# psklavos1/adaptive-city-nerf

Measured on AMD Instinct MI355X. Metric: ray-samples/sec + PSNR, 4096 rays×256 samples, 1/2/4/8 MI355X, higher is better.
Workload: dtype f32; 1 GPU; c2; samples_per_ray=256, parallelism=ray-sharded x1

## Files before the change

### adaptive_city_nerf_amd/csrc/render.hip

```cpp
#include "acn_device.h"
#include "acn_internal.h"

using namespace acn;

#ifndef ACN_MLP_F16X3
#define ACN_MLP_F16X3 1
#endif

#ifndef ACN_SLOTS
#define ACN_SLOTS 1
#endif

#ifndef ACN_XPAIR
#define ACN_XPAIR 2
#endif
#ifndef ACN_LEVEL_PARITY
#define ACN_LEVEL_PARITY 0
#endif
#ifndef ACN_FINE_POL
#define ACN_FINE_POL 0
#endif
#ifndef ACN_FINE_FROM
#define ACN_FINE_FROM 8
#endif
// ... 978 lines not shown
                   [&](int, float px, float py, float pz, const float (&shv)[8], uint32_t& folded, float& yr, float& yg,
                       float& yb, float& ys) {
                       container_tile<INTERP, ROUTE, FOLD>(cfg, W, px, py, pz, shv, cb, &folded, lane, yr, yg, yb, ys);
                   });
    }
}

#ifndef ACN_RENDER_WS
#define ACN_RENDER_WS 1
#endif
constexpr int kWsMaxS = 256;
#ifndef ACN_WS_CHECK
#define ACN_WS_CHECK 0
#endif
#ifndef ACN_WS_PREFOLD
#define ACN_WS_PREFOLD 1
#endif
#ifndef ACN_WS_DTILE
#define ACN_WS_DTILE (ACN_WS_CHECK ? 0 : 8)
#endif

__device__ __forceinline__ void composite_ray_lds(const RenderParams& p, const BgArgs& bg, int64_t ray,
                                                  const f32x4* __restrict__ ys, int lane, float step) {
    const int j = lane & 31, h = lane >> 5;
    const int S = p.S;
    const float* rq = p.rays + ray * 8;
    const float dx = rq[3], dy = rq[4], dz = rq[5];
    const float near = rq[6], far = rq[7];
    const float* jit = p.jitter ? p.jitter + ray * S : nullptr;
    RayAcc acc{1.0, 0.0f, 0.0f, 0.0f, 0.0f, 0.0f};
    for (int s0 = 0; s0 < S; s0 += 32) {
        const int s = s0 + j;
        const bool valid = s < S;
        const int sc = valid ? s : S - 1;
        float t, dist;
        if (!jit) {
            const int i0 = sc < S - 1 ? sc : S - 2;
            const float ta = tlin_sel(near, far, i0, S, step), tb = tlin_sel(near, far, i0 + 1, S, step);
            t = sc < S - 1 ? ta : tb;
            dist = tb - ta;
        } else {
            t = tval(near, far, sc, S, jit);
            const float tn = (sc < S - 1) ? tval(near, far, sc + 1, S, jit) : t;
            const float tp = (sc == S - 1 && S > 1) ? tval(near, far, sc - 1, S, jit) : t;
            dist = (sc < S - 1) ? (tn - t) : (t - tp);
        }
        const f32x4 y = ys[sc];
        const float cr = clamp_nan(y[0], 0.0f, 1.0f);
        const float cg = clamp_nan(y[1], 0.0f, 1.0f);
        const float cbl = clamp_nan(y[2], 0.0f, 1.0f);
        float sig = clamp_min_nan(y[3], 0.0f);
        if (p.sigma_scale != 1.0f) sig = sig * p.sigma_scale;
        float wv;
        composite_tile(acc, valid, cr, cg, cbl, sig, t, dist, j, &wv);
        if (p.weights && valid && h == 0) p.weights[ray * S + s] = wv;
    }
    float bgc[3];
    background(bg, dx, dy, dz, lane, bgc);
    float r, g, b, dd, a;
    finish_ray(acc, r, g, b, dd, a);
    if (lane == 0) {
        if (bg.mode != ACN_BG_NONE) {
            const float om = 1.0f - a;
            r = r + om * bgc[0];
            g = g + om * bgc[1];
            b = b + om * bgc[2];
        }
        p.rgb[ray * 3 + 0] = r;
        p.rgb[ray * 3 + 1] = g;
        p.rgb[ray * 3 + 2] = b;
        p.depth[ray] = dd;
        p.acc[ray] = a;
    }
}

template <int INTERP>
__global__ void __launch_bounds__(1024, 4) render_ws_kernel(FieldCfg cfg, BgArgs bg, RenderParams p) {
    constexpr bool FOLD = ACN_SHFOLD != 0;
    __shared__ __attribute__((aligned(16))) float smem[PK_FLOATS];
    __shared__ __attribute__((aligned(16))) float cbuf[FOLD ? 16 * 64 : 4];
    __shared__ __attribute__((aligned(16))) f32x4 ybuf[16 * kWsMaxS];
    __shared__ int qhead;
    __shared__ int done[16];
    stage_weights<1>(smem, p.packed);
    const float* W = smem;
    const int wave = __builtin_amdgcn_readfirstlane(threadIdx.x >> 6);
    float* cb = FOLD ? cbuf + wave * 64 : nullptr;
    const int S = p.S;
    const int T = (S + 31) >> 5;
    const float step = 1.0f / (float)(S - 1);
    int64_t base, hi, stride;
    if ((gridDim.x & 7) == 0) {
        const int64_t chunk = (p.N + 7) >> 3;
        const int64_t lo = min(p.N, (int64_t)(blockIdx.x & 7) * chunk);
        hi = min(p.N, lo + chunk);
        base = lo + (int64_t)(blockIdx.x >> 3) * 16;
        stride = (int64_t)(gridDim.x >> 3) * 16;
    } else {
        hi = p.N;
        base = (int64_t)blockIdx.x * 16;
        stride = (int64_t)gridDim.x * 16;
    }
    for (; base < hi; base += stride) {
        const int tid = opaque_v((int)threadIdx.x);
        const int lane = tid & 63, j = lane & 31, h = lane >> 5;
        const float kz = __int_as_float(opaque_s(0));
        const int nr = (int)min((int64_t)16, hi - base);
        if (tid == 0) qhead = 0;
        if (tid < 16) done[tid] = 0;
        constexpr bool PRE = FOLD && ACN_WS_PREFOLD;
        if (PRE && wave < nr) {
            const int64_t r0 = p.order ? (int64_t)__builtin_amdgcn_readfirstlane(p.order[base + wave]) : base + wave;
            const float* rp = p.rays + r0 * 8;
            float sh[16], sv[8];
            dir_sh(rp[3], rp[4], rp[5], sh, kz);
            sh_rows_for_half(sh, h, sv);
            fold_sh_bias(W, sv, lane, cbuf + wave * 64);
        }
        __syncthreads();
#if ACN_WS_DTILE
        static_assert(!ACN_WS_DTILE || (FOLD && ACN_WS_PREFOLD && !ACN_WS_CHECK), "depth tiles read the pre-folded bias");
        static_assert(16 % (ACN_WS_DTILE > 0 ? ACN_WS_DTILE : 1) == 0, "ACN_WS_DTILE: rays per tile divide 16");
        {
            constexpr int R = ACN_WS_DTILE, D = 32 / R, NG = 16 / R;
            const int ND = (S + D - 1) / D;
            const float shz[8] = {0.0f, 0.0f, 0.0f, 0.0f, 0.0f, 0.0f, 0.0f, 0.0f};
            int gcur = -1;
            int slot = 0;
            float ox = 0.0f, oy = 0.0f, oz = 0.0f, dx = 0.0f, dy = 0.0f, dz = 0.0f, near = 0.0f, far = 0.0f;
            const float* jit = nullptr;
            for (;;) {
                int item = 0;
                if (lane == 0) item = __hip_atomic_fetch_add(&qhead, 1, __ATOMIC_RELAXED, __HIP_MEMORY_SCOPE_WORKGROUP);
                item = __builtin_amdgcn_readlane(item, 0);
                if (item >= NG * ND) break;
                const int g = NG == 1 ? 0 : item % NG, q = NG == 1 ? item : item / NG;
                if (g != gcur) {
                    slot = g * R + (j % R);
                    const int ls = slot < nr ? slot : nr - 1;
                    const int64_t ray = p.order ? (int64_t)p.order[base + ls] : base + ls;
                    const float* rp = p.rays + ray * 8;
                    ox = rp[0], oy = rp[1], oz = rp[2], dx = rp[3], dy = rp[4], dz = rp[5];
                    near = rp[6], far = rp[7];
                    jit = p.jitter ? p.jitter + ray * S : nullptr;
                    gcur = g;
                }
                const int s = q * D + j / R;
                const int sc = s < S ? s : S - 1;
                float t;
                if (!jit) {
                    const int i0 = sc < S - 1 ? sc : S - 2;
                    const float ta = tlin_sel(near, far, i0, S, step), tb = tlin_sel(near, far, i0 + 1, S, step);
                    t = sc < S - 1 ? ta : tb;
                } else {
                    t = tval(near, far, sc, S, jit);
                }
                const float px = ox + dx * t, py = oy + dy * t, pz = oz + dz * t;
                uint32_t fl = 1u;
                float yr, yg, yb, ys;
                container_tile<INTERP, 0, FOLD>(cfg, W, px, py, pz, shz, cbuf + slot * 64, &fl, lane, yr, yg, yb, ys);
                if (h == 0 && s < S && slot < nr) {
                    f32x4 v;
                    v[0] = yr, v[1] = yg, v[2] = yb, v[3] = ys;
                    ybuf[slot * kWsMaxS + s] = v;
                }
            }
            __syncthreads();
            if (wave < nr) {
                const int64_t ray_w = p.order ? (int64_t)__builtin_amdgcn_readfirstlane(p.order[base + wave]) : base + wave;
                composite_ray_lds(p, bg, ray_w, ybuf + wave * kWsMaxS, lane, step);
            }
            __syncthreads();
            continue;
        }
#endif
        int64_t cur = -1;
        uint32_t folded = 0u;
        float shv[8] = {0.0f, 0.0f, 0.0f, 0.0f, 0.0f, 0.0f, 0.0f, 0.0f};
        float ox = 0.0f, oy = 0.0f, oz = 0.0f, dx = 0.0f, dy = 0.0f, dz = 0.0f, near = 0.0f, far = 0.0f;
        const float* jit = nullptr;
        for (;;) {
            int item = 0;
            if (lane == 0) item = __hip_atomic_fetch_add(&qhead, 1, __ATOMIC_RELAXED, __HIP_MEMORY_SCOPE_WORKGROUP);
            item = __builtin_amdgcn_readlane(item, 0);
            if (item >= nr * T) break;
            const int tile = item / nr, slot = item - tile * nr;
            const int64_t ray = p.order ? (int64_t)__builtin_amdgcn_readfirstlane(p.order[base + slot]) : base + slot;
            if (ray != cur) {
                const float* rp = p.rays + ray * 8;
                ox = rp[0], oy = rp[1], oz = rp[2], dx = rp[3], dy = rp[4], dz = rp[5];
                near = rp[6], far = rp[7];
                jit = p.jitter ? p.jitter + ray * S : nullptr;
                if (!PRE || ACN_WS_CHECK) {
                    float sh[16];
                    dir_sh(dx, dy, dz, sh, kz);
                    sh_rows_for_half(sh, h, shv);
                    if (!PRE) folded = 0u;
                }
                cur = ray;
            }
            if (PRE) {
                cb = cbuf + slot * 64;
                folded = 1u;
            }
            const int s = tile * 32 + j;
            const int sc = s < S ? s : S - 1;
            float t;
            if (!jit) {
                const int i0 = sc < S - 1 ? sc : S - 2;
                const float ta = tlin_sel(near, far, i0, S, step), tb = tlin_sel(near, far, i0 + 1, S, step);
                t = sc < S - 1 ? ta : tb;
            } else {
                t = tval(near, far, sc, S, jit);
            }
            const float px = ox + dx * t, py = oy + dy * t, pz = oz + dz * t;
            float yr, yg, yb, ys;
            container_tile<INTERP, 0, FOLD>(cfg, W, px, py, pz, shv, cb, &folded, lane, yr, yg, yb, ys);
#if ACN_WS_CHECK
            {
                float cr, cg, cbb, cs;
                field_tile<INTERP, false, true>(W, cfg.ex[0], cfg.log2T, px, py, pz, shv, nullptr, lane, cr, cg, cbb, cs);
                cs = trunc_exp(cs);
                if (__float_as_uint(cr) != __float_as_uint(yr) || __float_as_uint(cg) != __float_as_uint(yg) ||
                    __float_as_uint(cbb) != __float_as_uint(yb) || __float_as_uint(cs) != __float_as_uint(ys))
                    yr = __int_as_float(0x7fc00000);
            }
#endif
            if (h == 0 && s < S) {
                f32x4 v;
                v[0] = yr, v[1] = yg, v[2] = yb, v[3] = ys;
                ybuf[slot * kWsMaxS + s] = v;
            }
            int old = 0;
            if (lane == 0) old = __hip_atomic_fetch_add(&done[slot], 1, __ATOMIC_ACQ_REL, __HIP_MEMORY_SCOPE_WORKGROUP);
            old = __builtin_amdgcn_readlane(old, 0);
            if (old != T - 1) continue;
            composite_ray_lds(p, bg, ray, ybuf + slot * kWsMaxS, lane, step);
        }
        __syncthreads();
    }
}

#ifndef ACN_SLOTS_SINGLE
#define ACN_SLOTS_SINGLE 1
#endif
constexpr uint32_t kSingleRay = 1u << 31;
__device__ __forceinline__ void soft_route_bits(const FieldCfg& cfg, float px, float py, float pz, uint32_t& m,
                                                bool& exact) {
    float mins = INFINITY;
    for (int k = 0; k < cfg.K; ++k) mins = fminf(mins, route_dist2(cfg, k, px, py, pz));
    float mind = sqrtf(mins);
    mind = mind < 1e-6f ? 1e-6f : mind;
    const float thr = cfg.bm * mind, thr2 = route_thr2(thr);
// ... 973 lines not shown
    Keval = active_module >= 0 ? 1 : K;
    ACN_REQUIRE(workspace && workspace_bytes >= (size_t)Keval * PK_BYTES, "workspace too small: need %zu bytes",
                (size_t)Keval * PK_BYTES);
    ACN_REQUIRE(((uintptr_t)workspace & 15) == 0, "workspace must be 16-byte aligned");
    interp = experts[k0].interp;
    const int log2T = experts[k0].log2T;
    PackArgs pa{};
    for (int i = 0; i < Keval; ++i) {
        const acn_expert& e = experts[k0 + i];
        int st = check_expert(e, k0 + i);
        if (st) return st;
        if (e.interp != interp || e.log2T != log2T)
            return acn_set_error(ACN_ERR_UNSUPPORTED, "experts must share interpolation and log2_hashmap_size");
        ExpertMeta& m = cfg.ex[i];
        m.table = e.table;
        for (int a = 0; a < 3; ++a) {
            m.amin[a] = e.aabb_min[a];
            m.ext[a] = e.aabb_extent[a];
            m.rext[a] = 1.0f / e.aabb_extent[a];
        }
        for (int l = 0; l < 16; ++l) m.res[l] = e.res[l];
        pa.e[i] = PackSrc{e.sig_w0, e.sig_b0, e.sig_w1, e.sig_b1, e.sigh_w, e.sigh_b, e.geo_w, e.geo_b,
                          e.col_w0, e.col_b0, e.col_w1, e.col_b1, e.col_w2, e.col_b2};
    }
    cfg.K = Keval;
    cfg.log2T = log2T;
    cfg.cluster_2d = routing->cluster_2d;
    cfg.bm = routing->boundary_margin;
    if (active_module >= 0 || K == 1) cfg.routing = 0;
    else cfg.routing = routing->boundary_margin > 1.0f ? 1 : 2;
    for (int k = 0; k < K && active_module < 0; ++k)
        for (int a = 0; a < 3; ++a) cfg.cent[k][a] = routing->centroids[k][a];
    if (do_pack) {
        hipLaunchKernelGGL(pack_kernel, dim3((PK_FLOATS + 255) / 256, Keval), dim3(256), 0, s, pa, Keval,
                           (float*)workspace);
        return acn_check_launch("acn_pack_experts");
    }
    return ACN_OK;
}

}

#define ACN_DISPATCH_I(L, I)                                           \
    do {                                                               \
        if (cfg.routing == 0) L(I, 1, 0);                              \
        else if (cfg.routing == 1) { if (K == 2) L(I, 2, 1); else L(I, 0, 1); } \
        else { if (K == 2) L(I, 2, 2); else L(I, 0, 2); }              \
    } while (0)
#define ACN_DISPATCH(L)                                                \
    do {                                                               \
        if (interp == 1) ACN_DISPATCH_I(L, 1);                         \
        else if (interp == 0) ACN_DISPATCH_I(L, 0);                    \
        else ACN_DISPATCH_I(L, 2);                                     \
    } while (0)

__global__ void __launch_bounds__(256) sample_train_kernel(const float* __restrict__ rays, int64_t N, int S,
                                                           const float* __restrict__ jit, float3 amin, float3 ext,
                                                           float lo, float hi, float* __restrict__ t_out,
                                                           float* __restrict__ x01, float* __restrict__ sh_out) {
    const int64_t m = (int64_t)blockIdx.x * 256 + threadIdx.x;
    if (m >= N * (int64_t)S) return;
    const int64_t ray = m / S;
    const int s = (int)(m - ray * S);
    const float* rp = rays + ray * 8;
    const float ox = rp[0], oy = rp[1], oz = rp[2], dx = rp[3], dy = rp[4], dz = rp[5];
    const float t = tval(rp[6], rp[7], s, S, jit ? jit + ray * S : nullptr);
    t_out[m] = t;
    const float px = ox + dx * t, py = oy + dy * t, pz = oz + dz * t;
    x01[m * 3 + 0] = clamp_nan((px - amin.x) / ext.x, lo, hi);
    x01[m * 3 + 1] = clamp_nan((py - amin.y) / ext.y, lo, hi);
    x01[m * 3 + 2] = clamp_nan((pz - amin.z) / ext.z, lo, hi);
    float sh[16];
    dir_sh(dx, dy, dz, sh);
    float4* o4 = reinterpret_cast<float4*>(sh_out + m * 16);
#pragma unroll
    for (int q = 0; q < 4; ++q) o4[q] = make_float4(sh[4 * q], sh[4 * q + 1], sh[4 * q + 2], sh[4 * q + 3]);
}

#define ACN_ORDER_MAX 8192
#define ACN_ORDER_BINS 4096
#ifndef ACN_ORDER_COUNTING
#define ACN_ORDER_COUNTING 1
#endif
__device__ __forceinline__ uint32_t spread6(uint32_t v) {
    v &= 63u;
    v = (v | (v << 4)) & 0x30Fu;
    v = (v | (v << 2)) & 0x333u;
    v = (v | (v << 1)) & 0x555u;
    return v;
}
template <int OP>
__device__ __forceinline__ float wave_reduce(float v) {
    auto op = [](float a, float b) { return OP == 0 ? a + b : fmaxf(a, b); };
    v = op(v, __int_as_float(__builtin_amdgcn_update_dpp(0, __float_as_int(v), 0xB1, 0xF, 0xF, false)));
    v = op(v, __int_as_float(__builtin_amdgcn_update_dpp(0, __float_as_int(v), 0x4E, 0xF, 0xF, false)));
    v = op(v, __int_as_float(__builtin_amdgcn_update_dpp(0, __float_as_int(v), 0x141, 0xF, 0xF, false)));
    v = op(v, __int_as_float(__builtin_amdgcn_update_dpp(0, __float_as_int(v), 0x140, 0xF, 0xF, false)));
    const float r0 = __int_as_float(__builtin_amdgcn_readlane(__float_as_int(v), 0));
    const float r1 = __int_as_float(__builtin_amdgcn_readlane(__float_as_int(v), 16));
    const float r2 = __int_as_float(__builtin_amdgcn_readlane(__float_as_int(v), 32));
    const float r3 = __int_as_float(__builtin_amdgcn_readlane(__float_as_int(v), 48));
    return op(op(r0, r1), op(r2, r3));
}
template <int OP>
__device__ __forceinline__ void block_reduce3(float& a, float& b, float& c, float* red) {
    a = wave_reduce<OP>(a), b = wave_reduce<OP>(b), c = wave_reduce<OP>(c);
    const int w = threadIdx.x >> 6;
    if ((threadIdx.x & 63) == 0) red[w] = a, red[16 + w] = b, red[32 + w] = c;
    __syncthreads();
    a = red[0], b = red[16], c = red[32];
    for (int k = 1; k < 16; ++k) a += red[k], b += red[16 + k], c += red[32 + k];
    __syncthreads();
}
__device__ __forceinline__ void block_reduce4max(float& a, float& b, float& c, float& d, float* red) {
    a = wave_reduce<1>(a), b = wave_reduce<1>(b), c = wave_reduce<1>(c), d = wave_reduce<1>(d);
    const int w = threadIdx.x >> 6;
    if ((threadIdx.x & 63) == 0) red[w] = a, red[16 + w] = b, red[32 + w] = c, red[48 + w] = d;
    __syncthreads();
    for (int k = 0; k < 16; ++k)
        a = fmaxf(a, red[k]), b = fmaxf(b, red[16 + k]), c = fmaxf(c, red[32 + k]), d = fmaxf(d, red[48 + k]);
    __syncthreads();
}
__device__ __forceinline__ bool dir_ok(float x, float y, float z) {
    const float n2 = x * x + y * y + z * z;
    return n2 > 0.0f && n2 < 3.0e38f;
}
template <bool FINAL>
__device__ __forceinline__ void radix_pass6(const uint16_t* kin, const uint16_t* iin, int shift, int N, int* cnt,
                                            int* wsum, uint16_t* kout, uint16_t* iout, int32_t* __restrict__ order) {
    const int tid = threadIdx.x, w = tid >> 6, lane = tid & 63;
    const int B = (((N + 15) >> 4) + 63) & ~63;
    const int lo = w * B, hi = min(N, lo + B);
    cnt[tid] = 0;
    __syncthreads();
    for (int p0 = lo; p0 < hi; p0 += 64) {
        const int pos = p0 + lane;
        const bool v = pos < hi;
        const int dig = v ? (kin[pos] >> shift) & 63 : 0;
        const uint64_t m = same_digit_lanes(v, dig);
        if (v && lanes_below(m) == 0) cnt[dig * 16 + w] += __popcll(m);
    }
    __syncthreads();
    const int val = cnt[tid];
    const int incl = wave_incl_scan(val);
    if (lane == 63) wsum[w] = incl;
    __syncthreads();
    int base = incl - val;
    for (int k = 0; k < w; ++k) base += wsum[k];
    cnt[tid] = base;
    __syncthreads();
    for (int p0 = lo; p0 < hi; p0 += 64) {
        const int pos = p0 + lane;
        const bool v = pos < hi;
        const uint16_t key = v ? kin[pos] : (uint16_t)0;
        const int dig = (key >> shift) & 63;
        const uint64_t m = same_digit_lanes(v, dig);
        const int below = lanes_below(m);
        const int run = v ? cnt[dig * 16 + w] : 0;
        if (v) {
            const int dst = run + below;
            const int idx = iin ? (int)iin[pos] : pos;
            if (FINAL) {
                order[dst] = idx;
            } else {
                kout[dst] = key;
                iout[dst] = (uint16_t)idx;
            }
        }
        if (v && below == 0) cnt[dig * 16 + w] = run + __popcll(m);
    }
    __syncthreads();
}
__global__ void __launch_bounds__(1024) ray_order_kernel(const float* __restrict__ rays, int N,
                                                         int32_t* __restrict__ order) {
    constexpr int PER = ACN_ORDER_MAX / 1024;
    __shared__ int cnt[1024];
    __shared__ __attribute__((aligned(16))) float dir[3][ACN_ORDER_MAX];
    __shared__ uint16_t cell_of[ACN_ORDER_MAX];
    __shared__ int wsum[16];
    __shared__ float red[16 * 4];
    const int tid = threadIdx.x;
    float sx = 0.0f, sy = 0.0f, sz = 0.0f;
#pragma unroll
    for (int q = 0; q < PER; ++q) {
        const int i = tid + q * 1024;
        if (i < N) {
            const float* rp = rays + (int64_t)i * 8;
            const float x = rp[3], y = rp[4], z = rp[5];
            dir[0][i] = x, dir[1][i] = y, dir[2][i] = z;
            if (dir_ok(x, y, z)) {
                const float r = rsqrtf(x * x + y * y + z * z);
                sx += x * r, sy += y * r, sz += z * r;
            }
        }
    }
#if ACN_ORDER_DIAG == 3
    for (int i = tid; i < N; i += 1024) order[i] = i + (int)(sx * 0.0f);
    return;
#endif
    block_reduce3<0>(sx, sy, sz, red);
    const float mn = sqrtf(sx * sx + sy * sy + sz * sz);
    float mx = 0.0f, my = 0.0f, mz = 1.0f;
    if (mn > 0.0f && mn < 3.0e38f) mx = sx / mn, my = sy / mn, mz = sz / mn;
    float ax = 0.0f, ay = 0.0f, az = 0.0f;
    if (fabsf(mx) <= fabsf(my) && fabsf(mx) <= fabsf(mz)) ax = 1.0f;
    else if (fabsf(my) <= fabsf(mz)) ay = 1.0f;
    else az = 1.0f;
    float e1x = my * az - mz * ay, e1y = mz * ax - mx * az, e1z = mx * ay - my * ax;
    const float e1n = rsqrtf(e1x * e1x + e1y * e1y + e1z * e1z);
    e1x *= e1n, e1y *= e1n, e1z *= e1n;
    const float e2x = my * e1z - mz * e1y, e2y = mz * e1x - mx * e1z, e2z = mx * e1y - my * e1x;
    auto coords = [&](int i, float& u, float& v) -> bool {
        const float x = dir[0][i], y = dir[1][i], z = dir[2][i];
        if (!dir_ok(x, y, z)) return false;
        const float dm = x * mx + y * my + z * mz;
        if (!(dm > 0.0f)) return false;
        u = (x * e1x + y * e1y + z * e1z) / dm;
        v = (x * e2x + y * e2y + z * e2z) / dm;
        return fabsf(u) < 1.0e30f && fabsf(v) < 1.0e30f;
    };
    float umin = 3.0e38f, vmin = 3.0e38f, umax = -3.0e38f, vmax = -3.0e38f;
    float cu[PER], cv[PER];
    bool cok[PER];
#pragma unroll
    for (int q = 0; q < PER; ++q) {
        const int i = tid + q * 1024;
        cok[q] = i < N && coords(i, cu[q], cv[q]);
        if (cok[q]) umin = fminf(umin, cu[q]), umax = fmaxf(umax, cu[q]), vmin = fminf(vmin, cv[q]), vmax = fmaxf(vmax, cv[q]);
    }
#if ACN_ORDER_DIAG == 2
    for (int i = tid; i < N; i += 1024) order[i] = i + (int)(umin * 0.0f + umax * 0.0f);
    return;
#endif
#if ACN_ORDER_DIAG == 1
    umin = -2.0f, vmin = -2.0f, umax = 2.0f, vmax = 2.0f;
#else
    umin = -umin, vmin = -vmin;
    block_reduce4max(umin, vmin, umax, vmax, red);
    umin = -umin, vmin = -vmin;
#endif
    const float su = umax > umin ? 63.999f / (umax - umin) : 0.0f;
    const float sv = vmax > vmin ? 63.999f / (vmax - vmin) : 0.0f;
#pragma unroll
    for (int q = 0; q < PER; ++q) {
        const int i = tid + q * 1024;
        if (i >= N) break;
        int c = ACN_ORDER_BINS - 1;
        if (cok[q]) {
            const uint32_t qu = (uint32_t)fminf(fmaxf((cu[q] - umin) * su, 0.0f), 63.0f);
            const uint32_t qv = (uint32_t)fminf(fmaxf((cv[q] - vmin) * sv, 0.0f), 63.0f);
            c = (int)(spread6(qu) | (spread6(qv) << 1));
        }
        cell_of[i] = (uint16_t)c;
    }
    __syncthreads();
#if ACN_ORDER_COUNTING
    {
        constexpr int kOrderSlice = 64;
        int* bins = reinterpret_cast<int*>(&dir[2][0]);
        int* start = reinterpret_cast<int*>(&dir[1][0]);
        uint16_t* lst = reinterpret_cast<uint16_t*>(&dir[0][0]);
        __shared__ int maxc;
        if (tid == 0) maxc = 0;
        for (int b = tid; b < ACN_ORDER_BINS; b += 1024) bins[b] = 0;
        __syncthreads();
        int mloc = 0;
        for (int i = tid; i < N; i += 1024) {
            const int c = atomicAdd(&bins[cell_of[i]], 1) + 1;
            mloc = c > mloc ? c : mloc;
        }
        if (mloc > kOrderSlice) atomicMax(&maxc, mloc);
        __syncthreads();
        if (maxc == 0) {
            constexpr int BPT = ACN_ORDER_BINS / 1024;
            int c[BPT], tot = 0;
#pragma unroll
            for (int q = 0; q < BPT; ++q) tot += (c[q] = bins[tid * BPT + q]);
            const int lane = tid & 63, w = tid >> 6;
            const int incl = wave_incl_scan(tot);
            if (lane == 63) wsum[w] = incl;
            __syncthreads();
            int base = incl - tot;
            for (int k = 0; k < w; ++k) base += wsum[k];
#pragma unroll
            for (int q = 0; q < BPT; ++q) {
                start[tid * BPT + q] = base;
                bins[tid * BPT + q] = base;
                base += c[q];
            }
            __syncthreads();
            for (int i = tid; i < N; i += 1024) lst[atomicAdd(&bins[cell_of[i]], 1)] = (uint16_t)i;
            __syncthreads();
            for (int i = tid; i < N; i += 1024) {
                const int cl = cell_of[i], s0 = start[cl], s1 = bins[cl];
                int r = 0;
                for (int j = s0; j < s1; ++j) r += (int)lst[j] < i ? 1 : 0;
                order[s0 + r] = i;
            }
            return;
        }
        __syncthreads();
    }
#endif
    uint16_t* key1 = reinterpret_cast<uint16_t*>(&dir[0][0]);
    uint16_t* idx1 = reinterpret_cast<uint16_t*>(&dir[1][0]);
    radix_pass6<false>(cell_of, nullptr, 0, N, cnt, wsum, key1, idx1, nullptr);
    radix_pass6<true>(key1, idx1, 6, N, cnt, wsum, nullptr, nullptr, order);
}

extern "C" size_t acn_workspace_bytes(int K) { return (size_t)(K < 1 ? 1 : K) * PK_BYTES; }

extern "C" size_t acn_render_order_bytes(int64_t N) {
    if (N < 1) return 0;
    return N <= ACN_ORDER_MAX ? (size_t)N * sizeof(int32_t) : 0;
}

extern "C" int acn_ray_order(const float* rays, int64_t N, int32_t* order, void* stream) {
    ACN_REQUIRE(N >= 1 && N <= ACN_ORDER_MAX, "acn_ray_order: N must be in [1, %d], got %lld", ACN_ORDER_MAX,
                (long long)N);
    ACN_REQUIRE(rays && order, "acn_ray_order: NULL pointer");
    hipLaunchKernelGGL(ray_order_kernel, dim3(1), dim3(1024), 0, (hipStream_t)stream, rays, (int)N, order);
    return acn_check_launch("acn_ray_order");
}

extern "C" int acn_pack_experts(const acn_expert* experts, const acn_routing* routing, int active_module,
                                void* workspace, size_t workspace_bytes, void* stream) {
    FieldCfg cfg{};
    int interp, K;
    return prepare(experts, routing, active_module, workspace, workspace_bytes, (hipStream_t)stream, cfg, interp, K,
                   true);
}

extern "C" int acn_field_fwd(const float* x, int64_t M, int64_t ld, const acn_expert* experts,
                             const acn_routing* routing, int active_module, void* workspace, size_t workspace_bytes,
                             float* out, void* stream) {
    ACN_REQUIRE(M >= 0 && ld >= 6, "acn_field_fwd: x must be (N, D>=6)");
    if (M == 0) return ACN_OK;
    ACN_REQUIRE(x && out, "acn_field_fwd: NULL pointer");
    hipStream_t s = (hipStream_t)stream;
    FieldCfg cfg{};
    int interp, K;
    int st = prepare(experts, routing, active_module, workspace, workspace_bytes, s, cfg, interp, K, false);
    if (st) return st;
    FieldParams p{x, M, ld, (const float*)workspace, out};
    const int64_t ntiles = (M + 31) / 32;
    const int64_t wgs = (ntiles + 15) / 16;
    const dim3 grid((unsigned)(wgs < num_cus() ? wgs : num_cus())), block(1024);
#define ACN_FIELD_LAUNCH(I, KL, R) hipLaunchKernelGGL((field_kernel<I, KL, R>), grid, block, 0, s, cfg, p)
    ACN_DISPATCH(ACN_FIELD_LAUNCH);
#undef ACN_FIELD_LAUNCH
    return acn_check_launch("acn_field_fwd");
}

extern "C" int acn_render_stratified_fwd(const float* rays, int64_t N, int S, const float* jitter,
                                         const acn_expert* experts, const acn_routing* routing, int active_module,
                                         const acn_background* bg, float sigma_scale, float tau, void* workspace,
                                         size_t workspace_bytes, float* rgb, float* depth, float* weights, float* acc,
                                         void* stream) {
    return acn_render_stratified_fwd_ordered(rays, N, S, jitter, experts, routing, active_module, bg, sigma_scale, tau,
                                             workspace, workspace_bytes, rgb, depth, weights, acc, nullptr, 0, stream);
}

extern "C" int acn_render_stratified_fwd_ordered(const float* rays, int64_t N, int S, const float* jitter,
                                                 const acn_expert* experts, const acn_routing* routing,
                                                 int active_module, const acn_background* bg, float sigma_scale,
                                                 float tau, void* workspace, size_t workspace_bytes, float* rgb,
                                                 float* depth, float* weights, float* acc, void* order_scratch,
                                                 size_t order_bytes, void* stream) {
    ACN_REQUIRE(N >= 0, "acn_render_stratified_fwd: N must be >= 0");
    ACN_REQUIRE(S >= 2, "acn_render_stratified_fwd: ray_samples must be >= 2, got %d", S);
    if (N == 0) return ACN_OK;
    ACN_REQUIRE(rays && rgb && depth && acc, "acn_render_stratified_fwd: NULL pointer");
    ACN_REQUIRE(bg, "acn_render_stratified_fwd: NULL background");
    if (bg->mode == ACN_BG_MLP) {
        ACN_REQUIRE(bg->w1 && bg->b1 && bg->w2 && bg->b2, "background MLP pointers are NULL");
        ACN_REQUIRE(bg->hidden >= 1 && bg->hidden <= 64, "bg_hidden must be in [1, 64], got %d", bg->hidden);
    }
    hipStream_t s = (hipStream_t)stream;
    FieldCfg cfg{};
    int interp, K;
    int st = prepare(experts, routing, active_module, workspace, workspace_bytes, s, cfg, interp, K, false);
    if (st) return st;
    BgArgs b{bg->mode, bg->hidden, {bg->color[0], bg->color[1], bg->color[2]}, bg->w1, bg->b1, bg->w2, bg->b2};
    RenderParams p{rays, N, S, jitter, (const float*)workspace, sigma_scale, tau, rgb, depth, weights, acc, nullptr};
    int64_t wgs = (N + 15) / 16;
    if ((num_cus() & 7) == 0) wgs = (wgs + 7) & ~(int64_t)7;
    const dim3 grid((unsigned)(wgs < num_cus() ? wgs : num_cus())), block(1024);
    const bool slots = ACN_SLOTS && cfg.routing != 0 && K != 2;
    if (order_scratch && !slots && N <= ACN_ORDER_MAX && order_bytes >= (size_t)N * sizeof(int32_t)) {
        hipLaunchKernelGGL(ray_order_kernel, dim3(1), dim3(1024), 0, s, rays, (int)N, (int32_t*)order_scratch);
        p.order = (const int32_t*)order_scratch;
    }
    const bool wss = ACN_RENDER_WSS && S <= kWssMaxS(8) && !(tau > 0.0f);
    const bool wss16 = ACN_WSS_RAYS16 && S <= kWssMaxS(16);
#define ACN_RENDER_LAUNCH(I, KL, R)                                                                    \
    do {                                                                                              \
        if (ACN_SLOTS && KL == 0 && R != 0 && wss && wss16) hipLaunchKernelGGL((render_wss_kernel<I, (R == 0 ? 1 : R), 16>), grid, dim3(ACN_SLOTS_THREADS), 0, s, cfg, b, p); \
        else if (ACN_SLOTS && KL == 0 && R != 0 && wss) hipLaunchKernelGGL((render_wss_kernel<I, (R == 0 ? 1 : R), 8>), grid, dim3(ACN_SLOTS_THREADS), 0, s, cfg, b, p); \
        else if (ACN_SLOTS && KL == 0 && R != 0) hipLaunchKernelGGL((render_slots_kernel<I, (R == 0 ? 1 : R)>), grid, dim3(ACN_SLOTS_THREADS), 0, s, cfg, b, p); \
        else hipLaunchKernelGGL((render_kernel<I, KL, R>), grid, block, 0, s, cfg, b, p);            \
    } while (0)
    if (ACN_RENDER_WS && cfg.routing == 0 && S <= kWsMaxS && !(tau > 0.0f)) {
        if (interp == 1) hipLaunchKernelGGL(render_ws_kernel<1>, grid, block, 0, s, cfg, b, p);
        else if (interp == 0) hipLaunchKernelGGL(render_ws_kernel<0>, grid, block, 0, s, cfg, b, p);
        else hipLaunchKernelGGL(render_ws_kernel<2>, grid, block, 0, s, cfg, b, p);
        return acn_check_launch("acn_render_stratified_fwd");
    }
    ACN_DISPATCH(ACN_RENDER_LAUNCH);
#undef ACN_RENDER_LAUNCH
    return acn_check_launch("acn_render_stratified_fwd");
}

extern "C" int acn_volume_render_fwd(const float* rgb_sigma, const float* t_vals, const float* bg, int64_t N, int S,
                                     int raw_rgb, int raw_sigma, float sigma_scale, float* rgb, float* depth,
                                     float* weights, float* acc, void* stream) {
    ACN_REQUIRE(N >= 0 && S >= 2, "acn_volume_render_fwd: need N >= 0 and S >= 2 (got S=%d)", S);
    if (N == 0) return ACN_OK;
    ACN_REQUIRE(rgb_sigma && t_vals && rgb && depth && acc, "acn_volume_render_fwd: NULL pointer");
    const int64_t wgs = (N + 3) / 4;
    const dim3 grid((unsigned)(wgs < 4096 ? wgs : 4096)), block(256);
    hipLaunchKernelGGL(volume_render_kernel, grid, block, 0, (hipStream_t)stream, rgb_sigma, t_vals, bg, N, S, raw_rgb,
                       raw_sigma, sigma_scale, rgb, depth, weights, acc);
    return acn_check_launch("acn_volume_render_fwd");
}

extern "C" int acn_volume_render_bwd(const float* rgb_sigma, const float* t_vals, const float* bg, int64_t N, int S,
                                     float sigma_scale, const float* g_rgb, const float* g_depth,
                                     const float* g_weights, const float* g_acc, float* g_rgb_sigma, float* g_bg,
                                     void* stream) {
    ACN_REQUIRE(N >= 0 && S >= 2, "acn_volume_render_bwd: need N >= 0 and S >= 2 (got S=%d)", S);
    if (N == 0) return ACN_OK;
    ACN_REQUIRE(rgb_sigma && t_vals && g_rgb_sigma, "acn_volume_render_bwd: NULL pointer");
    ACN_REQUIRE(!g_bg || bg, "acn_volume_render_bwd: g_bg requested without bg");
    const int64_t wgs = (N + 3) / 4;
    const dim3 grid((unsigned)(wgs < 8192 ? wgs : 8192)), block(256);
    hipLaunchKernelGGL(volume_render_bwd_kernel, grid, block, 0, (hipStream_t)stream, rgb_sigma, t_vals, bg, N, S,
                       sigma_scale, g_rgb, g_depth, g_weights, g_acc, g_rgb_sigma, g_bg);
    return acn_check_launch("acn_volume_render_bwd");
}

extern "C" size_t acn_composite_mse_train_workspace_bytes(void) { return kCmMaxBlocks * sizeof(double) + 16; }

extern "C" int acn_routed_composite_mse_train(const float* rays, int64_t N, int S, const float* t_vals,
                                              const float* pair_out, const float* pair_w, const int32_t* pmap, int K,
                                              const int32_t* pidx, int64_t P, const int64_t* live,
                                              const acn_background* bg, const float* rgbs, const float* g_loss,
                                              float* rgb, float* dirs, float* g_bg, float* g_pair_out, float* loss,
                                              void* workspace, size_t workspace_bytes, void* stream) {
    ACN_REQUIRE(N >= 1 && S >= 2 && S <= kCmMaxS && K >= 1 && K <= ACN_MAX_EXPERTS && P >= 0 && bg,
                "acn_routed_composite_mse_train: bad sizes (N=%lld S=%d K=%d P=%lld)", (long long)N, S, K,
                (long long)P);
    ACN_REQUIRE(rays && t_vals && pmap && rgbs && g_loss && rgb && dirs && loss && workspace &&
                    (P == 0 || (pair_out && pair_w && pidx && g_pair_out)),
                "acn_routed_composite_mse_train: NULL pointer");
    ACN_REQUIRE(workspace_bytes >= acn_composite_mse_train_workspace_bytes(),
                "acn_routed_composite_mse_train: workspace too small");
    ACN_REQUIRE(((uintptr_t)pair_out & 15) == 0 && ((uintptr_t)g_pair_out & 15) == 0,
                "acn_routed_composite_mse_train: pair buffers must be 16-byte aligned");
    if (bg->mode == ACN_BG_MLP) {
        ACN_REQUIRE(bg->w1 && bg->b1 && bg->w2 && bg->b2, "background MLP pointers are NULL");
        ACN_REQUIRE(bg->hidden >= 1 && bg->hidden <= 64, "bg_hidden must be in [1, 64], got %d", bg->hidden);
    }
    BgArgs b{bg->mode, bg->hidden, {bg->color[0], bg->color[1], bg->color[2]}, bg->w1, bg->b1, bg->w2, bg->b2};
    int64_t wgs = (N + 3) / 4;
    wgs = wgs < kCmMaxBlocks ? wgs : kCmMaxBlocks;
    double* partials = (double*)workspace;
    unsigned int* counter = (unsigned int*)((char*)workspace + kCmMaxBlocks * sizeof(double));
    const size_t lds = (size_t)(kCmThreads / 64) * S * (sizeof(float4) + sizeof(float));
    hipLaunchKernelGGL(composite_mse_train_kernel, dim3((unsigned)wgs), dim3(kCmThreads), lds, (hipStream_t)stream, b,
                       rays, (const float4*)pair_out, pair_w, pmap, K, t_vals, rgbs, N, S, g_loss, rgb, dirs, g_bg,
                       (float4*)g_pair_out, pidx, live, P, partials, counter, loss);
    return acn_check_launch("acn_routed_composite_mse_train");
}
// ... 336 lines not shown
```

Before: 3.942 billion ray-samples/s.

## Restructure ray-ordering kernel into templated register-resident counting sort

Rewrites the single-block ray_order_kernel so it is templated on thread count and rays per thread. Ray directions now stay in registers instead of an LDS staging array. Bin counting is fused into the cell-computation loop, with each ray's arrival index packed into its key, and the prefix scan and rank loops use vectorised int4 LDS accesses. A launcher picks the smallest per-thread template for N, defaulting to 512 threads. A disabled-by-default diagnostic timing path is also added to the work-stealing render kernel. The aim is to cut the serial latency of this one-block preprocessing launch, though it is a small share of total render time.

```diff
diff --git a/adaptive_city_nerf_amd/csrc/render.hip b/adaptive_city_nerf_amd/csrc/render.hip
--- a/adaptive_city_nerf_amd/csrc/render.hip
+++ b/adaptive_city_nerf_amd/csrc/render.hip
@@ -1084,6 +1084,10 @@
     __shared__ __attribute__((aligned(16))) f32x4 ybuf[16 * kWsMaxS];
     __shared__ int qhead;
     __shared__ int done[16];
+#if ACN_DIAG_WSTIME
+    const uint32_t dw_entry = (uint32_t)__builtin_amdgcn_s_memrealtime();
+    uint32_t dw_first = 0u;
+#endif
     stage_weights<1>(smem, p.packed);
     const float* W = smem;
     const int wave = __builtin_amdgcn_readfirstlane(threadIdx.x >> 6);
@@ -1160,6 +1164,9 @@
                 const float px = ox + dx * t, py = oy + dy * t, pz = oz + dz * t;
                 uint32_t fl = 1u;
                 float yr, yg, yb, ys;
+#if ACN_DIAG_WSTIME
+                if (dw_first == 0u) dw_first = (uint32_t)__builtin_amdgcn_s_memrealtime() | 1u;
+#endif
                 container_tile<INTERP, 0, FOLD>(cfg, W, px, py, pz, shz, cbuf + slot * 64, &fl, lane, yr, yg, yb, ys);
                 if (h == 0 && s < S && slot < nr) {
                     f32x4 v;
@@ -1168,9 +1175,21 @@
                 }
             }
             __syncthreads();
+#if ACN_DIAG_WSTIME
+            const uint32_t dw_last = (uint32_t)__builtin_amdgcn_s_memrealtime();
+#endif
             if (wave < nr) {
                 const int64_t ray_w = p.order ? (int64_t)__builtin_amdgcn_readfirstlane(p.order[base + wave]) : base + wave;
                 composite_ray_lds(p, bg, ray_w, ybuf + wave * kWsMaxS, lane, step);
+#if ACN_DIAG_WSTIME
+                if (lane == 0) {
+                    p.rgb[ray_w * 3 + 0] = __int_as_float((int)dw_entry);
+                    p.rgb[ray_w * 3 + 1] = __int_as_float((int)dw_first);
+                    p.rgb[ray_w * 3 + 2] = __int_as_float((int)dw_last);
+                    p.depth[ray_w] = __int_as_float((int)(uint32_t)__builtin_amdgcn_s_memrealtime());
+                    p.acc[ray_w] = __int_as_float((int)blockIdx.x);
+                }
+#endif
             }
             __syncthreads();
             continue;
@@ -2310,6 +2329,9 @@
 #ifndef ACN_ORDER_COUNTING
 #define ACN_ORDER_COUNTING 1
 #endif
+#ifndef ACN_ORDER_THREADS
+#define ACN_ORDER_THREADS 512
+#endif
 __device__ __forceinline__ uint32_t spread6(uint32_t v) {
     v &= 63u;
     v = (v | (v << 4)) & 0x30Fu;
@@ -2330,34 +2352,33 @@
     const float r3 = __int_as_float(__builtin_amdgcn_readlane(__float_as_int(v), 48));
     return op(op(r0, r1), op(r2, r3));
 }
-template <int OP>
-__device__ __forceinline__ void block_reduce3(float& a, float& b, float& c, float* red) {
-    a = wave_reduce<OP>(a), b = wave_reduce<OP>(b), c = wave_reduce<OP>(c);
+template <int OP, int NW, int NV>
+__device__ __forceinline__ void block_reduce(float (&v)[NV], float* red) {
+#pragma unroll
+    for (int k = 0; k < NV; ++k) v[k] = wave_reduce<OP>(v[k]);
     const int w = threadIdx.x >> 6;
-    if ((threadIdx.x & 63) == 0) red[w] = a, red[16 + w] = b, red[32 + w] = c;
+    if ((threadIdx.x & 63) == 0) {
+#pragma unroll
+        for (int k = 0; k < NV; ++k) red[k * NW + w] = v[k];
+    }
     __syncthreads();
-    a = red[0], b = red[16], c = red[32];
-    for (int k = 1; k < 16; ++k) a += red[k], b += red[16 + k], c += red[32 + k];
-    __syncthreads();
-}
-__device__ __forceinline__ void block_reduce4max(float& a, float& b, float& c, float& d, float* red) {
-    a = wave_reduce<1>(a), b = wave_reduce<1>(b), c = wave_reduce<1>(c), d = wave_reduce<1>(d);
-    const int w = threadIdx.x >> 6;
-    if ((threadIdx.x & 63) == 0) red[w] = a, red[16 + w] = b, red[32 + w] = c, red[48 + w] = d;
-    __syncthreads();
-    for (int k = 0; k < 16; ++k)
-        a = fmaxf(a, red[k]), b = fmaxf(b, red[16 + k]), c = fmaxf(c, red[32 + k]), d = fmaxf(d, red[48 + k]);
-    __syncthreads();
+#pragma unroll
+    for (int k = 0; k < NV; ++k) {
+        float a = red[k * NW];
+#pragma unroll
+        for (int j = 1; j < NW; ++j) a = OP == 0 ? a + red[k * NW + j] : fmaxf(a, red[k * NW + j]);
+        v[k] = a;
+    }
 }
 __device__ __forceinline__ bool dir_ok(float x, float y, float z) {
     const float n2 = x * x + y * y + z * z;
     return n2 > 0.0f && n2 < 3.0e38f;
 }
-template <bool FINAL>
+template <int NW, bool FINAL>
 __device__ __forceinline__ void radix_pass6(const uint16_t* kin, const uint16_t* iin, int shift, int N, int* cnt,
                                             int* wsum, uint16_t* kout, uint16_t* iout, int32_t* __restrict__ order) {
     const int tid = threadIdx.x, w = tid >> 6, lane = tid & 63;
-    const int B = (((N + 15) >> 4) + 63) & ~63;
+    const int B = (((N + NW - 1) / NW) + 63) & ~63;
     const int lo = w * B, hi = min(N, lo + B);
     cnt[tid] = 0;
     __syncthreads();
@@ -2366,7 +2387,7 @@
         const bool v = pos < hi;
         const int dig = v ? (kin[pos] >> shift) & 63 : 0;
         const uint64_t m = same_digit_lanes(v, dig);
-        if (v && lanes_below(m) == 0) cnt[dig * 16 + w] += __popcll(m);
+        if (v && lanes_below(m) == 0) cnt[dig * NW + w] += __popcll(m);
     }
     __syncthreads();
     const int val = cnt[tid];
@@ -2384,7 +2405,7 @@
         const int dig = (key >> shift) & 63;
         const uint64_t m = same_digit_lanes(v, dig);
         const int below = lanes_below(m);
-        const int run = v ? cnt[dig * 16 + w] : 0;
+        const int run = v ? cnt[dig * NW + w] : 0;
         if (v) {
             const int dst = run + below;
             const int idx = iin ? (int)iin[pos] : pos;
@@ -2395,38 +2416,50 @@
                 iout[dst] = (uint16_t)idx;
             }
         }
-        if (v && below == 0) cnt[dig * 16 + w] = run + __popcll(m);
+        if (v && below == 0) cnt[dig * NW + w] = run + __popcll(m);
     }
     __syncthreads();
 }
-__global__ void __launch_bounds__(1024) ray_order_kernel(const float* __restrict__ rays, int N,
-                                                         int32_t* __restrict__ order) {
-    constexpr int PER = ACN_ORDER_MAX / 1024;
-    __shared__ int cnt[1024];
-    __shared__ __attribute__((aligned(16))) float dir[3][ACN_ORDER_MAX];
+template <int NT, int PER>
+__global__ void __launch_bounds__(NT) ray_order_kernel(const float* __restrict__ rays, int N,
+                                                       int32_t* __restrict__ order) {
+    static_assert(NT * PER <= ACN_ORDER_MAX && ACN_ORDER_BINS % (4 * NT) == 0 && PER <= 32, "ray_order_kernel shape");
+    constexpr int NW = NT / 64;
+    constexpr int BPT = ACN_ORDER_BINS / NT;
+    constexpr int kOrderSlice = 64;
+    __shared__ __attribute__((aligned(16))) int bins[ACN_ORDER_BINS + 64];
+    __shared__ __attribute__((aligned(16))) int start[ACN_ORDER_BINS];
+    __shared__ uint16_t lst[ACN_ORDER_MAX];
     __shared__ uint16_t cell_of[ACN_ORDER_MAX];
-    __shared__ int wsum[16];
-    __shared__ float red[16 * 4];
+    __shared__ int cnt[NT];
+    __shared__ int wsum[NW];
+    __shared__ float red_sum[3 * NW], red_box[4 * NW];
+    __shared__ int big;
     const int tid = threadIdx.x;
-    float sx = 0.0f, sy = 0.0f, sz = 0.0f;
+    float x[PER], y[PER], z[PER];
 #pragma unroll
     for (int q = 0; q < PER; ++q) {
-        const int i = tid + q * 1024;
-        if (i < N) {
-            const float* rp = rays + (int64_t)i * 8;
-            const float x = rp[3], y = rp[4], z = rp[5];
-            dir[0][i] = x, dir[1][i] = y, dir[2][i] = z;
-            if (dir_ok(x, y, z)) {
-                const float r = rsqrtf(x * x + y * y + z * z);
-                sx += x * r, sy += y * r, sz += z * r;
-            }
-        }
+        const int i = tid + q * NT;
+        const float* rp = rays + (int64_t)(i < N ? i : N - 1) * 8;
+        const float lx = rp[3], ly = rp[4], lz = rp[5];
+        x[q] = i < N ? lx : 0.0f, y[q] = i < N ? ly : 0.0f, z[q] = i < N ? lz : 0.0f;
+    }
+    for (int b = tid * 4; b < ACN_ORDER_BINS; b += NT * 4) *reinterpret_cast<int4*>(&bins[b]) = make_int4(0, 0, 0, 0);
+    if (tid < 64) bins[ACN_ORDER_BINS + tid] = 0;
+    if (tid == 0) big = 0;
+    float s[3] = {0.0f, 0.0f, 0.0f};
+#pragma unroll
+    for (int q = 0; q < PER; ++q) {
+        const bool ok = dir_ok(x[q], y[q], z[q]);
+        const float r = rsqrtf(x[q] * x[q] + y[q] * y[q] + z[q] * z[q]);
+        s[0] += ok ? x[q] * r : 0.0f, s[1] += ok ? y[q] * r : 0.0f, s[2] += ok ? z[q] * r : 0.0f;
     }
 #if ACN_ORDER_DIAG == 3
-    for (int i = tid; i < N; i += 1024) order[i] = i + (int)(sx * 0.0f);
+    for (int i = tid; i < N; i += NT) order[i] = i + (int)(s[0] * 0.0f);
     return;
 #endif
-    block_reduce3<0>(sx, sy, sz, red);
+    block_reduce<0, NW, 3>(s, red_sum);
+    const float sx = s[0], sy = s[1], sz = s[2];
     const float mn = sqrtf(sx * sx + sy * sy + sz * sz);
     float mx = 0.0f, my = 0.0f, mz = 1.0f;
     if (mn > 0.0f && mn < 3.0e38f) mx = sx / mn, my = sy / mn, mz = sz / mn;
@@ -2438,102 +2471,124 @@
     const float e1n = rsqrtf(e1x * e1x + e1y * e1y + e1z * e1z);
     e1x *= e1n, e1y *= e1n, e1z *= e1n;
     const float e2x = my * e1z - mz * e1y, e2y = mz * e1x - mx * e1z, e2z = mx * e1y - my * e1x;
-    auto coords = [&](int i, float& u, float& v) -> bool {
-        const float x = dir[0][i], y = dir[1][i], z = dir[2][i];
-        if (!dir_ok(x, y, z)) return false;
-        const float dm = x * mx + y * my + z * mz;
-        if (!(dm > 0.0f)) return false;
-        u = (x * e1x + y * e1y + z * e1z) / dm;
-        v = (x * e2x + y * e2y + z * e2z) / dm;
-        return fabsf(u) < 1.0e30f && fabsf(v) < 1.0e30f;
-    };
-    float umin = 3.0e38f, vmin = 3.0e38f, umax = -3.0e38f, vmax = -3.0e38f;
-    float cu[PER], cv[PER];
-    bool cok[PER];
+    float box[4] = {-3.0e38f, -3.0e38f, -3.0e38f, -3.0e38f};
+    uint32_t okm = 0u;
 #pragma unroll
     for (int q = 0; q < PER; ++q) {
-        const int i = tid + q * 1024;
-        cok[q] = i < N && coords(i, cu[q], cv[q]);
-        if (cok[q]) umin = fminf(umin, cu[q]), umax = fmaxf(umax, cu[q]), vmin = fminf(vmin, cv[q]), vmax = fmaxf(vmax, cv[q]);
+        const float dx = x[q], dy = y[q], dz = z[q];
+        const float dm = dx * mx + dy * my + dz * mz;
+        const float rdm = __builtin_amdgcn_rcpf(dm);
+        const float u = (dx * e1x + dy * e1y + dz * e1z) * rdm;
+        const float v = (dx * e2x + dy * e2y + dz * e2z) * rdm;
+        const bool ok = dir_ok(dx, dy, dz) && dm > 0.0f && fabsf(u) < 1.0e30f && fabsf(v) < 1.0e30f;
+        okm |= ok ? 1u << q : 0u;
+        box[0] = ok ? fmaxf(box[0], -u) : box[0], box[1] = ok ? fmaxf(box[1], -v) : box[1];
+        box[2] = ok ? fmaxf(box[2], u) : box[2], box[3] = ok ? fmaxf(box[3], v) : box[3];
+        x[q] = ok ? u : 0.0f, y[q] = ok ? v : 0.0f;
     }
 #if ACN_ORDER_DIAG == 2
-    for (int i = tid; i < N; i += 1024) order[i] = i + (int)(umin * 0.0f + umax * 0.0f);
+    for (int i = tid; i < N; i += NT) order[i] = i + (int)(box[0] * 0.0f + box[2] * 0.0f);
     return;
 #endif
 #if ACN_ORDER_DIAG == 1
-    umin = -2.0f, vmin = -2.0f, umax = 2.0f, vmax = 2.0f;
+    const float umin = -2.0f, vmin = -2.0f, umax = 2.0f, vmax = 2.0f;
 #else
-    umin = -umin, vmin = -vmin;
-    block_reduce4max(umin, vmin, umax, vmax, red);
-    umin = -umin, vmin = -vmin;
+    block_reduce<1, NW, 4>(box, red_box);
+    const float umin = -box[0], vmin = -box[1], umax = box[2], vmax = box[3];
 #endif
     const float su = umax > umin ? 63.999f / (umax - umin) : 0.0f;
     const float sv = vmax > vmin ? 63.999f / (vmax - vmin) : 0.0f;
+    uint32_t kr[PER];
+    int mloc = 0;
 #pragma unroll
     for (int q = 0; q < PER; ++q) {
-        const int i = tid + q * 1024;
-        if (i >= N) break;
-        int c = ACN_ORDER_BINS - 1;
-        if (cok[q]) {
-            const uint32_t qu = (uint32_t)fminf(fmaxf((cu[q] - umin) * su, 0.0f), 63.0f);
-            const uint32_t qv = (uint32_t)fminf(fmaxf((cv[q] - vmin) * sv, 0.0f), 63.0f);
-            c = (int)(spread6(qu) | (spread6(qv) << 1));
-        }
-        cell_of[i] = (uint16_t)c;
-    }
+        const int i = tid + q * NT;
+        const uint32_t qu = (uint32_t)fminf(fmaxf((x[q] - umin) * su, 0.0f), 63.0f);
+        const uint32_t qv = (uint32_t)fminf(fmaxf((y[q] - vmin) * sv, 0.0f), 63.0f);
+        const uint32_t c = (okm >> q) & 1u ? spread6(qu) | (spread6(qv) << 1) : ACN_ORDER_BINS - 1;
+        const int arrival = atomicAdd(&bins[i < N ? (int)c : ACN_ORDER_BINS + (tid & 63)], 1);
+        kr[q] = c | ((uint32_t)arrival << 12);
+        mloc = i < N && arrival >= mloc ? arrival + 1 : mloc;
+    }
+    if (!ACN_ORDER_COUNTING || mloc > kOrderSlice) big = 1;
     __syncthreads();
-#if ACN_ORDER_COUNTING
-    {
-        constexpr int kOrderSlice = 64;
-        int* bins = reinterpret_cast<int*>(&dir[2][0]);
-        int* start = reinterpret_cast<int*>(&dir[1][0]);
-        uint16_t* lst = reinterpret_cast<uint16_t*>(&dir[0][0]);
-        __shared__ int maxc;
-        if (tid == 0) maxc = 0;
-        for (int b = tid; b < ACN_ORDER_BINS; b += 1024) bins[b] = 0;
+    if (big == 0) {
+        int c[BPT], tot = 0;
+#pragma unroll
+        for (int k = 0; k < BPT; k += 4) {
+            const int4 v = *reinterpret_cast<const int4*>(&bins[tid * BPT + k]);
+            c[k] = v.x, c[k + 1] = v.y, c[k + 2] = v.z, c[k + 3] = v.w;
+            tot += v.x + v.y + v.z + v.w;
+        }
+        const int lane = tid & 63, w = tid >> 6;
+        const int incl = wave_incl_scan(tot);
+        if (lane == 63) wsum[w] = incl;
         __syncthreads();
-        int mloc = 0;
-        for (int i = tid; i < N; i += 1024) {
-            const int c = atomicAdd(&bins[cell_of[i]], 1) + 1;
-            mloc = c > mloc ? c : mloc;
-        }
-        if (mloc > kOrderSlice) atomicMax(&maxc, mloc);
+        int base = incl - tot;
+        for (int k = 0; k < w; ++k) base += wsum[k];
+#pragma unroll
+        for (int k = 0; k < BPT; k += 4) {
+            int4 v;
+            v.x = base, v.y = v.x + c[k], v.z = v.y + c[k + 1], v.w = v.z + c[k + 2];
+            base = v.w + c[k + 3];
+            *reinterpret_cast<int4*>(&start[tid * BPT + k]) = v;
+        }
         __syncthreads();
-        if (maxc == 0) {
-            constexpr int BPT = ACN_ORDER_BINS / 1024;
-            int c[BPT], tot = 0;
-#pragma unroll
-            for (int q = 0; q < BPT; ++q) tot += (c[q] = bins[tid * BPT + q]);
-            const int lane = tid & 63, w = tid >> 6;
-            const int incl = wave_incl_scan(tot);
-            if (lane == 63) wsum[w] = incl;
-            __syncthreads();
-            int base = incl - tot;
-            for (int k = 0; k < w; ++k) base += wsum[k];
-#pragma unroll
-            for (int q = 0; q < BPT; ++q) {
-                start[tid * BPT + q] = base;
-                bins[tid * BPT + q] = base;
-                base += c[q];
-            }
-            __syncthreads();
-            for (int i = tid; i < N; i += 1024) lst[atomicAdd(&bins[cell_of[i]], 1)] = (uint16_t)i;
-            __syncthreads();
-            for (int i = tid; i < N; i += 1024) {
-                const int cl = cell_of[i], s0 = start[cl], s1 = bins[cl];
-                int r = 0;
-                for (int j = s0; j < s1; ++j) r += (int)lst[j] < i ? 1 : 0;
-                order[s0 + r] = i;
-            }
-            return;
+#pragma unroll
+        for (int q = 0; q < PER; ++q) {
+            const int i = tid + q * NT;
+            const uint32_t cl = kr[q] & (ACN_ORDER_BINS - 1);
+            const int s0 = start[cl];
+            if (i < N) lst[s0 + (int)(kr[q] >> 12)] = (uint16_t)i;
+            kr[q] = cl | ((uint32_t)s0 << 12);
         }
         __syncthreads();
-    }
-#endif
-    uint16_t* key1 = reinterpret_cast<uint16_t*>(&dir[0][0]);
-    uint16_t* idx1 = reinterpret_cast<uint16_t*>(&dir[1][0]);
-    radix_pass6<false>(cell_of, nullptr, 0, N, cnt, wsum, key1, idx1, nullptr);
-    radix_pass6<true>(key1, idx1, 6, N, cnt, wsum, nullptr, nullptr, order);
+        int nr[PER], steps = 0;
+#pragma unroll
+        for (int q = 0; q < PER; ++q) {
+            const int i = tid + q * NT;
+            nr[q] = i < N ? bins[kr[q] & (ACN_ORDER_BINS - 1)] : 0;
+            steps = nr[q] > steps ? nr[q] : steps;
+        }
+        int rank[PER];
+#pragma unroll
+        for (int q = 0; q < PER; ++q) rank[q] = 0;
+        for (int k = 0; k < steps; ++k) {
+#pragma unroll
+            for (int q = 0; q < PER; ++q) {
+                const int i = tid + q * NT;
+                const bool in = k < nr[q];
+                const int member = (int)lst[in ? (int)(kr[q] >> 12) + k : 0];
+                rank[q] += in && member < i ? 1 : 0;
+            }
+        }
+#pragma unroll
+        for (int q = 0; q < PER; ++q) {
+            const int i = tid + q * NT;
+            if (i < N) order[(int)(kr[q] >> 12) + rank[q]] = i;
+        }
+        return;
+    }
+#pragma unroll
+    for (int q = 0; q < PER; ++q) {
+        const int i = tid + q * NT;
+        if (i < N) cell_of[i] = (uint16_t)(kr[q] & (ACN_ORDER_BINS - 1));
+    }
+    __syncthreads();
+    uint16_t* key1 = reinterpret_cast<uint16_t*>(&bins[0]);
+    uint16_t* idx1 = reinterpret_cast<uint16_t*>(&start[0]);
+    radix_pass6<NW, false>(cell_of, nullptr, 0, N, cnt, wsum, key1, idx1, nullptr);
+    radix_pass6<NW, true>(key1, idx1, 6, N, cnt, wsum, nullptr, nullptr, order);
+}
+
+static void launch_ray_order(const float* rays, int N, int32_t* order, hipStream_t s) {
+    constexpr int NT = ACN_ORDER_THREADS, PMAX = ACN_ORDER_MAX / NT;
+    if (N <= NT * (PMAX / 8))
+        hipLaunchKernelGGL((ray_order_kernel<NT, PMAX / 8>), dim3(1), dim3(NT), 0, s, rays, N, order);
+    else if (N <= NT * (PMAX / 2))
+        hipLaunchKernelGGL((ray_order_kernel<NT, PMAX / 2>), dim3(1), dim3(NT), 0, s, rays, N, order);
+    else
+        hipLaunchKernelGGL((ray_order_kernel<NT, PMAX>), dim3(1), dim3(NT), 0, s, rays, N, order);
 }
 
 extern "C" size_t acn_workspace_bytes(int K) { return (size_t)(K < 1 ? 1 : K) * PK_BYTES; }
@@ -2547,7 +2602,7 @@
     ACN_REQUIRE(N >= 1 && N <= ACN_ORDER_MAX, "acn_ray_order: N must be in [1, %d], got %lld", ACN_ORDER_MAX,
                 (long long)N);
     ACN_REQUIRE(rays && order, "acn_ray_order: NULL pointer");
-    hipLaunchKernelGGL(ray_order_kernel, dim3(1), dim3(1024), 0, (hipStream_t)stream, rays, (int)N, order);
+    launch_ray_order(rays, (int)N, order, (hipStream_t)stream);
     return acn_check_launch("acn_ray_order");
 }
 
@@ -2616,7 +2671,7 @@
     const dim3 grid((unsigned)(wgs < num_cus() ? wgs : num_cus())), block(1024);
     const bool slots = ACN_SLOTS && cfg.routing != 0 && K != 2;
     if (order_scratch && !slots && N <= ACN_ORDER_MAX && order_bytes >= (size_t)N * sizeof(int32_t)) {
-        hipLaunchKernelGGL(ray_order_kernel, dim3(1), dim3(1024), 0, s, rays, (int)N, (int32_t*)order_scratch);
+        launch_ray_order(rays, (int)N, (int32_t*)order_scratch, s);
         p.order = (const int32_t*)order_scratch;
     }
     const bool wss = ACN_RENDER_WSS && S <= kWssMaxS(8) && !(tau > 0.0f);
```

Result: no change. 3.972 billion ray-samples/s, median of 6 (+0.8%).
